# QZ1-boy/FCVSR

Measured on AMD Instinct MI355X. Metric: SR frames/sec (7-frame window, 4x 180x320->720x1280) + PSNR vs ref, higher is better.
Workload: dtype bf16

## Files before the change

### fcvsr_amd/csrc/convblk.hip

```cpp
#include "common.h"

namespace fcvsr {

constexpr int kCbT = 16;

template <int K>
__global__ __launch_bounds__(256) void convblk_conv_kernel(const float4* x, const float* __restrict__ w1,
                                                           const float* __restrict__ w2, const float* slope_p, float4* u,
                                                           float4* partial, int H, int W, int tiles_x, int tiles_y) {
  constexpr int P = K / 2;
  constexpr int XS = kCbT + 4 * P, TT = kCbT + 2 * P;
  __shared__ float4 xs[XS * XS];
  __shared__ float4 ts[TT * TT];
  __shared__ float4 red[256];
  const int tid = threadIdx.x;
  const int n = blockIdx.y;
  const int ty0 = (blockIdx.x / tiles_x) * kCbT, tx0 = (blockIdx.x % tiles_x) * kCbT;
  const float4* xn = x + (long long)n * H * W;
  const float slope = slope_p[0];
  for (int idx = tid; idx < XS * XS; idx += 256) {
    const int yy = idx / XS, xx = idx - yy * XS;
    const int gy = ty0 - 2 * P + yy, gx = tx0 - 2 * P + xx;
    float4 v = make_float4(0.f, 0.f, 0.f, 0.f);
    if (gy >= 0 && gy < H && gx >= 0 && gx < W) v = xn[(long long)gy * W + gx];
// ... 98 lines not shown
    gate_s[tid] = 1.f / (1.f + expf(-a));
  }
  __syncthreads();
  const long long pix = (long long)blockIdx.x * 256 + tid;
  if (pix >= HW) return;
  const int dir = bn / B, b = bn - dir * B;
  const float4 uu = u[(long long)bn * HW + pix];
  const float4 ss = sim[(long long)b * HW + pix];
  const float o0 = fmaf(uu.x, gate_s[0], uu.x) * ss.x;
  const float o1 = fmaf(uu.y, gate_s[1], uu.y) * ss.y;
  const float o2 = fmaf(uu.z, gate_s[2], uu.z) * ss.z;
  const float o3 = fmaf(uu.w, gate_s[3], uu.w) * ss.w;
  float* px = spec + ((long long)b * HW + pix) * ps;
  const int gi = (g0 + dir * g_stride) * 2;
  if (((ps | re_off | im_off) & 1) == 0 && (reinterpret_cast<uintptr_t>(spec) & 7) == 0) {
    *reinterpret_cast<float2*>(px + re_off + gi) = make_float2(o0, o1);
    *reinterpret_cast<float2*>(px + im_off + gi) = make_float2(o2, o3);
  } else {
    px[re_off + gi] = o0;
    px[re_off + gi + 1] = o1;
    px[im_off + gi] = o2;
    px[im_off + gi + 1] = o3;
  }
}

template <int K>
static void launch_convblk_conv(dim3 grid, hipStream_t st, const float4* x, const float* w1, const float* w2, const float* slope,
                                float4* u, float4* partial, int H, int W, int tx, int ty) {
  hipLaunchKernelGGL(convblk_conv_kernel<K>, grid, dim3(256), 0, st, x, w1, w2, slope, u, partial, H, W, tx, ty);
}

}

using namespace fcvsr;

extern "C" int fcvsr_convblk(const float* x, const float* w1, const float* w2, const float* prelu_slope, int ksize,
                             const float* ca_w1, const float* ca_w2, const float* sim, int B, int ndir, int H, int Wf,
                             float* u_scratch, float* partial_scratch, int64_t partial_elems, float* spec, int64_t pix_stride,
                             int re_off, int im_off, int g_stride, int g0, void* stream) {
  FCVSR_CHECK_ARG(x && w1 && w2 && prelu_slope && ca_w1 && ca_w2 && sim && u_scratch && partial_scratch && spec, "null pointer");
  FCVSR_CHECK_ARG(B > 0 && ndir > 0 && H > 0 && Wf > 0, "bad sizes");
  FCVSR_CHECK_ARG(ksize % 2 == 1 && ksize >= 1 && ksize <= 11, "kernel size: odd, 1..11");
  FCVSR_CHECK_ARG(((uintptr_t)x % 16) == 0 && ((uintptr_t)u_scratch % 16) == 0 && ((uintptr_t)sim % 16) == 0 &&
                      ((uintptr_t)partial_scratch % 16) == 0, "16-byte alignment");
  const int tx = cdiv(Wf, kCbT), ty = cdiv(H, kCbT);
  const int nblk = tx * ty, N = ndir * B;
  FCVSR_CHECK_ARG(partial_elems >= 4ll * N * nblk, "partial scratch too small");
  hipStream_t st = (hipStream_t)stream;
  dim3 grid(nblk, N);
  const float4* x4 = (const float4*)x;
  float4* u4 = (float4*)u_scratch;
  float4* p4 = (float4*)partial_scratch;
  switch (ksize) {
    case 1: launch_convblk_conv<1>(grid, st, x4, w1, w2, prelu_slope, u4, p4, H, Wf, tx, ty); break;
    case 3: launch_convblk_conv<3>(grid, st, x4, w1, w2, prelu_slope, u4, p4, H, Wf, tx, ty); break;
    case 5: launch_convblk_conv<5>(grid, st, x4, w1, w2, prelu_slope, u4, p4, H, Wf, tx, ty); break;
    case 7: launch_convblk_conv<7>(grid, st, x4, w1, w2, prelu_slope, u4, p4, H, Wf, tx, ty); break;
    case 9: launch_convblk_conv<9>(grid, st, x4, w1, w2, prelu_slope, u4, p4, H, Wf, tx, ty); break;
    default: launch_convblk_conv<11>(grid, st, x4, w1, w2, prelu_slope, u4, p4, H, Wf, tx, ty); break;
  }
  FCVSR_LAUNCH_CHECK();
  const long long HW = (long long)H * Wf;
  hipLaunchKernelGGL(convblk_tail_kernel2, dim3(cdiv(HW, 256), N), dim3(256), 0, st, (const float4*)u4, (const float4*)p4, nblk,
                     1.0f / (float)HW, ca_w1, ca_w2, (const float4*)sim, B, HW, spec, (long long)pix_stride, re_off, im_off,
                     g_stride, g0);
  FCVSR_LAUNCH_CHECK();
  return 0;
}
```

### fcvsr_amd/csrc/freq_head.hip

```cpp
#include "common.h"
#include "mfma_util.h"

namespace fcvsr {

constexpr int kFhPix = 128, kFhLD = 64 + 8;

struct FreqHeadArgs {
  const void* x;
  long long sx;
  float* out;
  int npix;
  const uint16_t* w0;
  const uint16_t* w1;
  const uint16_t* wl;
};

template <bool SRC_F32, int NHID>
__global__ __launch_bounds__(256, 4) void freq_head_kernel(FreqHeadArgs a) {
  __shared__ __align__(16) uint16_t A_s[kFhPix * kFhLD];
  __shared__ __align__(16) uint16_t B_s[64 * kFhLD];
  const int tid = threadIdx.x;
  const int lane = tid & 63, wave = tid >> 6;
  const int r = lane & 31, h = lane >> 5;
  const int flat0 = blockIdx.x * kFhPix;
  const int npix = a.npix;
  f32x16_t acc[2];
  auto zero_acc = [&]() {
#pragma unroll
    for (int nf = 0; nf < 2; ++nf)
#pragma unroll
      for (int i = 0; i < 16; ++i) acc[nf][i] = 0.f;
  };
  auto stage_w = [&](const uint16_t* w, int cin_pad, int c0, int rows) {
    uint4 v[2];
#pragma unroll
    for (int u = 0; u < 2; ++u) {
      const int row = (tid >> 3) + 32 * u;
      v[u] = make_uint4(0, 0, 0, 0);
      if (row < rows) v[u] = *reinterpret_cast<const uint4*>(w + (long long)row * cin_pad + c0 + (tid & 7) * 8);
    }
#pragma unroll
    for (int u = 0; u < 2; ++u) *reinterpret_cast<uint4*>(B_s + ((tid >> 3) + 32 * u) * kFhLD + (tid & 7) * 8) = v[u];
  };
  auto mma_chunk = [&](const uint16_t* prow, int ntile) {
    const uint16_t* wrow = B_s + r * kFhLD + h * 8;
#pragma unroll
    for (int kk = 0; kk < 4; ++kk) {
      const uint4 pf = *reinterpret_cast<const uint4*>(prow + kk * 16);
#pragma unroll
      for (int nf = 0; nf < 2; ++nf)
        if (nf < ntile) acc[nf] = mfma<true>(*reinterpret_cast<const uint4*>(wrow + nf * 32 * kFhLD + kk * 16), pf, acc[nf]);
    }
  };
  auto store_hidden = [&]() {
    uint16_t* trow = A_s + (wave * 32 + r) * kFhLD;
#pragma unroll
    for (int nf = 0; nf < 2; ++nf)
#pragma unroll
      for (int g = 0; g < 4; ++g) {
        const float4 v = make_float4(fmaxf(acc[nf][4 * g], 0.f), fmaxf(acc[nf][4 * g + 1], 0.f), fmaxf(acc[nf][4 * g + 2], 0.f),
                                     fmaxf(acc[nf][4 * g + 3], 0.f));
        *reinterpret_cast<uint2*>(trow + nf * 32 + 8 * g + 4 * h) = cvt4<true>(v);
      }
  };

  zero_acc();
  for (int c0 = 0; c0 < 128; c0 += 64) {
    __syncthreads();
    if (SRC_F32) {
      const int q = tid & 15, p0 = tid >> 4;
      const float* sb = reinterpret_cast<const float*>(a.x) + c0 + q * 4;
      float4 v[8];
#pragma unroll
      for (int i = 0; i < 8; ++i) {
        int pix = flat0 + p0 + i * 16;
        pix = pix < npix ? pix : npix - 1;
        v[i] = *reinterpret_cast<const float4*>(sb + (long long)pix * a.sx);
      }
#pragma unroll
      for (int i = 0; i < 8; ++i) *reinterpret_cast<uint2*>(A_s + (p0 + i * 16) * kFhLD + q * 4) = cvt4<true>(v[i]);
    } else {
      const int q = tid & 7, p0 = tid >> 3;
      const uint16_t* sb = reinterpret_cast<const uint16_t*>(a.x) + c0 + q * 8;
      uint4 v[4];
#pragma unroll
      for (int i = 0; i < 4; ++i) {
        int pix = flat0 + p0 + i * 32;
        pix = pix < npix ? pix : npix - 1;
        v[i] = *reinterpret_cast<const uint4*>(sb + (long long)pix * a.sx);
      }
#pragma unroll
      for (int i = 0; i < 4; ++i) *reinterpret_cast<uint4*>(A_s + (p0 + i * 32) * kFhLD + q * 8) = v[i];
    }
    stage_w(a.w0, 128, c0, 64);
    __syncthreads();
    mma_chunk(A_s + (wave * 32 + r) * kFhLD + h * 8, 2);
  }
  __syncthreads();
  store_hidden();

  if (NHID == 2) {
    zero_acc();
    __syncthreads();
    stage_w(a.w1, 64, 0, 64);
    __syncthreads();
    mma_chunk(A_s + (wave * 32 + r) * kFhLD + h * 8, 2);
    __builtin_amdgcn_wave_barrier();
    store_hidden();
  }

  zero_acc();
  __syncthreads();
  stage_w(a.wl, 64, 0, 32);
  __syncthreads();
  mma_chunk(A_s + (wave * 32 + r) * kFhLD + h * 8, 1);
  const int pix = flat0 + wave * 32 + r;
  if (h == 0 && pix < npix)
    *reinterpret_cast<float4*>(a.out + (long long)pix * 4) = make_float4(acc[0][0], acc[0][1], acc[0][2], acc[0][3]);
}

}

using namespace fcvsr;

extern "C" int fcvsr_freq_head(const void* x, int x_dtype, int64_t x_pix_stride, int64_t npix, const void* w0, const void* w_mid,
                               const void* w_last, float* out, void* stream) {
  FCVSR_CHECK_ARG(x && w0 && w_last && out, "null argument");
  FCVSR_CHECK_ARG(x_dtype == FCVSR_F32 || x_dtype == FCVSR_BF16, "x: f32 or bf16");
  FCVSR_CHECK_ARG(npix > 0 && npix < (1ll << 30) && x_pix_stride >= 128 && x_pix_stride % 8 == 0, "bad sizes / strides");
  FCVSR_CHECK_ARG(((uintptr_t)x % 16) == 0 && ((uintptr_t)w0 % 16) == 0 && ((uintptr_t)w_last % 16) == 0 &&
                      ((uintptr_t)out % 16) == 0 && (w_mid == nullptr || ((uintptr_t)w_mid % 16) == 0), "16-byte alignment");
  FreqHeadArgs a;
  a.x = x; a.sx = x_pix_stride; a.out = out; a.npix = (int)npix;
  a.w0 = (const uint16_t*)w0; a.w1 = (const uint16_t*)w_mid; a.wl = (const uint16_t*)w_last;
  dim3 grid(cdiv(npix, kFhPix));
  hipStream_t st = (hipStream_t)stream;
  if (x_dtype == FCVSR_F32) {
    if (w_mid) hipLaunchKernelGGL((freq_head_kernel<true, 2>), grid, dim3(256), 0, st, a);
    else hipLaunchKernelGGL((freq_head_kernel<true, 1>), grid, dim3(256), 0, st, a);
  } else {
    if (w_mid) hipLaunchKernelGGL((freq_head_kernel<false, 2>), grid, dim3(256), 0, st, a);
    else hipLaunchKernelGGL((freq_head_kernel<false, 1>), grid, dim3(256), 0, st, a);
  }
  FCVSR_LAUNCH_CHECK();
  return 0;
}
```

### fcvsr_amd/csrc/freq_mlp.hip

```cpp
#include "common.h"
#include "mfma_util.h"

namespace fcvsr {

constexpr int kFmC = 128;
constexpr int kFmPix = 128;
constexpr int kFmLD = 64 + 8;
constexpr int kFmTD = kFmC + 8;
constexpr int kFmTBytes = kFmPix * kFmTD * 2;
constexpr int kFmBBytes = kFmC * kFmLD * 2;
constexpr int kFmLds = kFmTBytes + kFmBBytes;

struct FreqMlpArgs {
  const float* xa[2];
  const float* xb[2];
  uint16_t* dst[2];
  long long sx, dsx;
  int npix, n_groups, tiles_per_group;
  const uint16_t* w0;
  const uint16_t* w2;
  const uint16_t* w4;
};

__global__ __launch_bounds__(256, 3) void freq_mlp3_kernel(FreqMlpArgs a) {
  extern __shared__ __align__(16) unsigned char lds[];
  uint16_t* T_s = reinterpret_cast<uint16_t*>(lds);
  uint16_t* A_s = T_s;
  uint16_t* B_s = reinterpret_cast<uint16_t*>(lds + kFmTBytes);
  const int tid = threadIdx.x;
  const int lane = tid & 63, wave = tid >> 6;
  const int r = lane & 31, h = lane >> 5;
  const int gi = blockIdx.x / a.tiles_per_group;
  const int flat0 = (blockIdx.x - gi * a.tiles_per_group) * kFmPix;
  const float* xa = a.xa[gi];
  const float* xb = a.xb[gi];
  const int npix = a.npix;

  f32x16_t acc[4];
  auto zero_acc = [&]() {
#pragma unroll
    for (int nf = 0; nf < 4; ++nf)
#pragma unroll
      for (int i = 0; i < 16; ++i) acc[nf][i] = 0.f;
  };
  auto mma_chunk = [&](const uint16_t* prow) {
    const uint16_t* wrow = B_s + r * kFmLD + h * 8;
#pragma unroll
    for (int kk = 0; kk < 4; ++kk) {
      const uint4 pf = *reinterpret_cast<const uint4*>(prow + kk * 16);
      uint4 wf[4];
#pragma unroll
      for (int nf = 0; nf < 4; ++nf) wf[nf] = *reinterpret_cast<const uint4*>(wrow + nf * 32 * kFmLD + kk * 16);
#pragma unroll
      for (int nf = 0; nf < 4; ++nf) acc[nf] = mfma<true>(wf[nf], pf, acc[nf]);
      if (kk & 1) __builtin_amdgcn_sched_barrier(0);
    }
// ... 138 lines not shown
                      dst_pix_stride >= kFmC && dst_pix_stride % 8 == 0, "bad sizes / strides");
  FCVSR_CHECK_ARG(npix * src_pix_stride * 4 < (1ll << 32) && npix * dst_pix_stride * 2 < (1ll << 32), "tensor too large for 32-bit offsets");
  FCVSR_CHECK_ARG(((uintptr_t)w0 % 16) == 0 && ((uintptr_t)w2 % 16) == 0 && ((uintptr_t)w4 % 16) == 0, "weights 16-byte aligned");
  FreqMlpArgs a;
  for (int d = 0; d < 2; ++d) {
    const int s = d < n_dirs ? d : 0;
    FCVSR_CHECK_ARG(xa[s] && xb[s] && dst[s] && ((uintptr_t)xa[s] % 16) == 0 && ((uintptr_t)xb[s] % 16) == 0 &&
                        ((uintptr_t)dst[s] % 16) == 0, "spectra / destination must be 16-byte aligned");
    a.xa[d] = xa[s]; a.xb[d] = xb[s]; a.dst[d] = (uint16_t*)dst[s];
  }
  a.sx = src_pix_stride; a.dsx = dst_pix_stride; a.npix = (int)npix; a.n_groups = n_dirs;
  a.tiles_per_group = cdiv(npix, kFmPix);
  a.w0 = (const uint16_t*)w0; a.w2 = (const uint16_t*)w2; a.w4 = (const uint16_t*)w4;
  static DevOnce attr;
  {
    hipError_t e = once_per_device(attr, [&] {
      return hipFuncSetAttribute((const void*)freq_mlp3_kernel, hipFuncAttributeMaxDynamicSharedMemorySize, kFmLds);
    });
    if (e != hipSuccess) {
      set_error("fcvsr_freq_mlp3: %s", hipGetErrorString(e));
      return (int)e;
    }
  }
  hipLaunchKernelGGL(freq_mlp3_kernel, dim3(a.tiles_per_group * n_dirs), dim3(256), kFmLds, (hipStream_t)stream, a);
  FCVSR_LAUNCH_CHECK();
  return 0;
}
```

### fcvsr_amd/engine.py

```python
from __future__ import annotations

import ctypes as C
import math
import weakref
from collections import OrderedDict
from typing import Dict, List, Optional, Tuple

import numpy as np
import torch

from . import hip
from .hip import ACT_LEAKY, ACT_NONE, ACT_PRELU, ACT_RELU, check, lib, ptr, stream_ptr, view


_MASKS: Dict[Tuple[int, int, int], torch.Tensor] = {}


def band_masks_half(Q: int, H: int, W: int) -> torch.Tensor:
    key = (Q, H, W)
    if key not in _MASKS:
        n = 1024
        step = math.sqrt((n / 2) ** 2 + (n / 2) ** 2) / Q
        d2 = (np.arange(-(n // 2), n - n // 2, 1) ** 2).astype(np.float64)
        r2 = np.power(np.sqrt(d2[:, None] + d2[None, :]), 2)
# ... 259 lines not shown
            cv = view(corr)
            check(L.fcvsr_corr_lookup(x1f.data_ptr(), x2f.data_ptr(), fs, B, H, Wf, 2 * n, 4, Wf, C.byref(cv), st),
                  "fcvsr_corr_lookup")
            for d in range(2):
                self._conv("MGAA.convcorr.0", [off[d * B:(d + 1) * B], corr], c0[d * B:(d + 1) * B], act=ACT_RELU, freq=True)
            self._conv("MGAA.convcorr.2", [c0], c1, act=ACT_RELU, freq=True)
            self._conv("MGAA.convcorr.4", [c1], off4, freq=True)
        else:
            if fused:
                check(L.fcvsr_freq_head(off.data_ptr(), hip.BF16, 2 * n, 2 * B * H * Wf,
                                        self._weights("MGAA.convcorr.0", torch.bfloat16, cols=(0, 2 * n))[0].data_ptr(),
                                        self._weights("MGAA.convcorr.2", torch.bfloat16)[0].data_ptr(),
                                        self._weights("MGAA.convcorr.4", torch.bfloat16)[0].data_ptr(), off4.data_ptr(), st),
                      "fcvsr_freq_head(convcorr)")
            else:
                c0 = self._new(dev, 2 * B, H, Wf, n, dtype=fdt)
                c1 = self._new(dev, 2 * B, H, Wf, n, dtype=fdt)
                self._conv("MGAA.convcorr.0", [off], c0, act=ACT_RELU, freq=True, cols=(0, 2 * n))
            xs = min(Wf, 8)
            corr = self._new(dev, B, H, xs, 84)
            cv = view(corr)
            check(L.fcvsr_corr_lookup(x1f.data_ptr(), x2f.data_ptr(), fs, B, H, Wf, 2 * n, 4, xs, C.byref(cv), st),
                  "fcvsr_corr_lookup")
            off_s = off[:, :, :xs].to(torch.float32, memory_format=torch.contiguous_format)
            c0_s = self._new(dev, 2 * B, H, xs, n, dtype=fdt)
            for d in range(2):
                self._conv("MGAA.convcorr.0", [off_s[d * B:(d + 1) * B], corr], c0_s[d * B:(d + 1) * B], act=ACT_RELU,
                           freq=True)
            if fused:
                c1_s = self._new(dev, 2 * B, H, xs, n, dtype=fdt)
                off4_s = self._new(dev, 2 * B, H, xs, 4)
                self._conv("MGAA.convcorr.2", [c0_s], c1_s, act=ACT_RELU, freq=True)
                self._conv("MGAA.convcorr.4", [c1_s], off4_s, freq=True)
                off4[:, :, :xs].copy_(off4_s)
            else:
                c0[:, :, :xs].copy_(c0_s)
                self._conv("MGAA.convcorr.2", [c0], c1, act=ACT_RELU, freq=True)
                self._conv("MGAA.convcorr.4", [c1], off4, freq=True)

        ospec = self._new(dev, B, H, Wf, 8 * A)
        u = self._new(dev, 2 * B, H, Wf, 4)
        ntile = ((H + 15) // 16) * ((Wf + 15) // 16)
        partial = self._new(dev, 2 * B * ntile * 4)
        for i in range(A):
            pre = f"MGAA.MConvB.{i}"
            w1 = self._weights(pre + ".conv1", "direct")[0]
            w2 = self._weights(pre + ".conv2", "direct")[0]
            check(L.fcvsr_convblk(off4.data_ptr(), w1.data_ptr(), w2.data_ptr(), par[pre + ".relu.weight"].data_ptr(),
                                  par[pre + ".conv1.weight"].shape[-1], par[pre + ".CA.conv_du.0.weight"].data_ptr(),
                                  par[pre + ".CA.conv_du.2.weight"].data_ptr(), sim.data_ptr(), B, 2, H, Wf, u.data_ptr(),
                                  partial.data_ptr(), partial.numel(), ospec.data_ptr(), 8 * A, 0, 4 * A, A, i, st),
                  "fcvsr_convblk")
        offsets = self._new(dev, B, H, W, 4 * A)
        ov = view(offsets)
        check(L.fcvsr_irfft2(ospec.data_ptr(), 8 * A, 4 * A, 0, B, H, W, 4 * A, None, None, C.byref(ov), st),
              "fcvsr_irfft2")

        kp = self._new(dev, B, H, W, n, dtype=self._adt())
        k0 = self._new(dev, B, H, W, n, dtype=self._adt())
        fused_iac = n % 32 == 0
        self._conv("MGAA.conv_KP", [x2], kp)
        self._conv("MGAA.F.0", [kp], k0)
        fold_f1 = fused_iac and n == 64 and self.precision != "f32" and self._model().fold_f1
        if not fold_f1:
            K = self._new(dev, B, H, W, A * 3 * n, dtype=self._adt() if fused_iac else torch.float32)
            self._conv("MGAA.F.1", [k0], K)

        fdt_act = x1.dtype
        al = self._new(dev, B, H, W, 2 * n, dtype=fdt_act)
        ping = [self._new(dev, B, H, W, n, dtype=fdt_act), self._new(dev, B, H, W, n, dtype=fdt_act)]
        if not fused_iac:
            if fdt_act != torch.float32:
                raise RuntimeError("16-bit activations need the fused IAC kernel (n_features % 32 == 0)")
            s = self._new(dev, B, H, W, n)
            vbuf = self._new(dev, B, H, W, n)
# ... 520 lines not shown
```

### fcvsr_amd/hip.py

```python
from __future__ import annotations

import ctypes as C
import os
from typing import Optional, Sequence

import numpy as np
import torch

_HERE = os.path.dirname(os.path.abspath(__file__))
LIB_PATH = os.path.join(_HERE, "lib", "libfcvsr_hip.so")

F32, BF16, F16, U8, U16 = 0, 1, 2, 3, 4
ACT_NONE, ACT_RELU, ACT_LEAKY, ACT_PRELU = 0, 1, 2, 3
_DT = {torch.float32: F32, torch.bfloat16: BF16, torch.float16: F16, torch.uint8: U8, torch.uint16: U16}


class View(C.Structure):
    _fields_ = [("ptr", C.c_void_p), ("sb", C.c_int64), ("sy", C.c_int64), ("sx", C.c_int64), ("sc", C.c_int64),
                ("c", C.c_int32), ("dtype", C.c_int32)]


class GcFinishLevel(C.Structure):
    _fields_ = [("partial", C.c_void_p), ("add", C.c_void_p), ("nparts", C.c_int32)]

# ... 62 lines not shown
    "fcvsr_last_conv_kernel": [],
    "fcvsr_conv2d_wgrad_scratch_elems": [C.c_int] * 7,
    "fcvsr_conv2d_wgrad": [C.c_void_p, C.c_void_p, C.c_int, C.c_int, C.c_int, C.c_int, C.c_int, C.c_int, C.c_int, C.c_void_p, C.c_void_p,
                           C.c_longlong, C.c_int, C.c_void_p],
    "fcvsr_conv2d_wgrad_mfma_eligible": [C.c_int] * 6,
    "fcvsr_conv2d_wgrad_mfma_scratch_elems": [C.c_int] * 7,
    "fcvsr_conv2d_wgrad_mfma": [C.c_void_p, C.c_void_p, C.c_int, C.c_int, C.c_int, C.c_int, C.c_int, C.c_int, C.c_int, C.c_void_p, C.c_void_p,
                                C.c_void_p, C.c_longlong, C.c_int, C.c_int, C.c_void_p],
    "fcvsr_abi_version": [],
    "fcvsr_device_count": [],
    "fcvsr_conv2d": [C.POINTER(ConvDesc), _VP],
    "fcvsr_conv2d_f32mfma": [C.POINTER(ConvDesc), _VP],
    "fcvsr_conv2d_f32mfma_eligible": [C.POINTER(ConvDesc)],
    "fcvsr_conv2d_mfma": [C.POINTER(ConvDesc), _I, _I, _VP],
    "fcvsr_conv2d_mfma_plan": [C.POINTER(ConvDesc), _I, _I, _I, _I, C.c_char_p, _I],
    "fcvsr_rfft2": [_PV, _I, _I, _I, _I, _VP, _I64, _I, _I, _VP],
    "fcvsr_irfft2": [_VP, _I64, _I, _I, _I, _I, _I, _I, _VP, _VP, _PV, _VP],
    "fcvsr_irfft2_bands": [_VP, _I64, _I, _I, _I, _I, _I, _I, _VP, _I, _VP, _PV, _VP],
    "fcvsr_corr_lookup": [_VP, _VP, _I64, _I, _I, _I, _I, _I, _I, _PV, _VP],
    "fcvsr_channel_sum": [_PV, _I, _I, _I, _VP, _VP, _I64, _VP],
    "fcvsr_ca_gate": [_VP, _F, _VP, _VP, _I, _I, _I, _VP, _VP],
    "fcvsr_convblk_tail": [_VP, _VP, _VP, _I, _I, _I, _I, _VP, _I64, _I, _I, _I, _I, _VP],
    "fcvsr_convblk": [_VP, _VP, _VP, _VP, _I, _VP, _VP, _VP, _I, _I, _I, _I, _VP, _VP, _I64, _VP, _I64, _I, _I, _I, _I, _VP],
    "fcvsr_warp": [_PV, _PV, _I, _I, _I, _PV, _VP],
    "fcvsr_sac_v": [_PV, _PV, _I, _I, _I, _PV, _VP],
    "fcvsr_sac_h": [_PV, _PV, _PV, _F, _I, _I, _I, _PV, _VP],
    "fcvsr_iac_step": [_PV, _PV, _PV, _PV, _F, _I, _I, _I, _PV, _VP],
    "fcvsr_feat_extract": [_PV, _I, _I, _I, _VP, _VP, _I, _VP, _VP, _VP, _I, _VP],
    "fcvsr_freq_head": [_VP, _I, _I64, _I64, _VP, _VP, _VP, _VP, _VP],
    "fcvsr_freq_mlp3": [_VP, _VP, _I, _I64, _I64, _VP, _VP, _VP, _VP, _I64, _VP],
    "fcvsr_iac_step2": [_PV, _PV, _PV, _PV, _F, _I, _I, _I, _PV, _VP],
    "fcvsr_iac_step2_fused": [_PV, _PV, _PV, _VP, _VP, _PV, _F, _I, _I, _I, _PV, _VP],
    "fcvsr_divenh": [_I, _I, _VP, _VP, _VP, _VP, _VP, _VP, _F, _VP, _VP, _VP, _VP, _I64, _I, _I, _I, _I, _VP],
    "fcvsr_divenh_apply_next": [_I, _VP, _VP, _VP, _VP, _VP, _VP, _F, _VP, _VP, _VP, _VP, _VP, _VP, _VP, _I64, _I, _I, _I, _I, _VP],
    "fcvsr_divenh_stage": [C.POINTER(DivEnhStageArgs), _VP],
    "fcvsr_scale_add": [_VP, _VP, _VP, _I, _VP, _I, _I, _I, _I, _I, _VP],
    "fcvsr_gc_context": [_VP, _VP, _VP, _VP, _I, _I, _I, _I, _VP, _VP, _I64, _VP],
    "fcvsr_gc_finish": [_VP, _I, _VP, _VP, _I, _I, _VP, _VP],
    "fcvsr_gc_apply": [_VP, _VP, _VP, _VP, _I, _F, _I, _I, _I, _I, _VP],
    "fcvsr_xscale": [_VP, _VP, _F, _VP, _VP, _VP, _I, _I, _I, _I, _I, _VP],
    "fcvsr_gc_finish_levels": [C.POINTER(GcFinishLevel), _I, _VP, _VP, _I, _I, _VP],
    "fcvsr_gc_partial_levels": [C.POINTER(GcPartialLevel), _I, _I, _VP, _I, _VP],
    "fcvsr_gc_apply_levels": [C.POINTER(GcApplyLevel), _I, _I, _I, _F, _I, _VP],
    "fcvsr_xscale_levels": [C.POINTER(XscaleLevel), _I, _I, _I, _VP],
    "fcvsr_rcb_level0": [_VP, _VP, _VP, _VP, _VP, _VP, _VP, _F, _F, _I, _I, _I, _I, _I, _VP],
    "fcvsr_rcb_tail": [C.POINTER(RcbTailArgs), _F, _I, _I, _VP],
    "fcvsr_pixel_shuffle": [_VP, _VP, _I, _I, _I, _I, _VP],
    "fcvsr_pixel_shuffle16": [_VP, _PV, _I, _I, _I, _I, _VP],
    "fcvsr_bilinear_up4": [_PV, _I, _I, _I, _PV, _VP],
    "fcvsr_tail_fused": [_PV, _VP, _VP, _VP, _VP, _VP, _I, _I, _I, _PV, _VP],
    "fcvsr_tail_fused_base": [_PV, _VP, _VP, _VP, _VP, _VP, _PV, _I, _I, _I, _PV, _VP],
    "fcvsr_conv_last": [_PV, _VP, _VP, _I, _I, _I, _I, _PV, _VP],
# ... 347 lines not shown
```

### include/fcvsr_hip.h

```cpp
#ifndef FCVSR_HIP_H
#define FCVSR_HIP_H

#include <stddef.h>
#include <stdint.h>

#ifdef __cplusplus
extern "C" {
#endif

#define FCVSR_ABI_VERSION 2

enum { FCVSR_E_ARG = -1, FCVSR_E_UNSUPPORTED = -2, FCVSR_E_NOGPU = -3 };
enum { FCVSR_F32 = 0, FCVSR_BF16 = 1, FCVSR_F16 = 2 };
enum { FCVSR_U8 = 3 };
enum { FCVSR_U16 = 4 };
enum { FCVSR_ACT_NONE = 0, FCVSR_ACT_RELU = 1, FCVSR_ACT_LEAKY = 2, FCVSR_ACT_PRELU = 3 };

typedef struct fcvsr_view {
  void*   ptr;
  int64_t sb, sy, sx, sc;
  int32_t c;
  int32_t dtype;
} fcvsr_view;

// ... 85 lines not shown
int fcvsr_rfft2(const fcvsr_view* src, int B, int H, int W, int n,
                float* spec, int64_t pix_stride, int im_off, int re_off, void* stream);
int fcvsr_irfft2(const float* spec, int64_t pix_stride, int im_off, int re_off, int B, int H, int W, int n,
                 const float* mask, float* work, const fcvsr_view* dst, void* stream);
int fcvsr_irfft2_bands(const float* spec, int64_t pix_stride, int im_off, int re_off, int B, int H, int W, int n,
                       const float* masks, int n_bands, float* work, const fcvsr_view* dst, void* stream);

int fcvsr_feat_extract(const fcvsr_view* x, int B, int H, int W, const void* w, const float* bias, int n_blk,
                       void* const* dst, const int64_t* dst_pix_stride, const int32_t* dst_ch_off, int dst_dtype,
                       void* stream);

int fcvsr_corr_lookup(const float* x1f, const float* x2f, int64_t pix_stride, int B, int H, int Wf, int C, int radius,
                      int x_count, const fcvsr_view* dst, void* stream);
int fcvsr_channel_sum(const fcvsr_view* src, int B, int H, int W, float* out, float* scratch, int64_t scratch_elems,
                      void* stream);
int fcvsr_ca_gate(const float* sum, float inv_hw, const float* w1, const float* w2, int B, int c, int cr,
                  float* gate, void* stream);
int fcvsr_convblk_tail(const float* u, const float* gate, const float* sim, int B, int ndir, int H, int Wf,
                       float* spec, int64_t pix_stride, int re_off, int im_off, int g_stride, int g0, void* stream);
int fcvsr_convblk(const float* x, const float* w1, const float* w2, const float* prelu_slope, int ksize, const float* ca_w1,
                  const float* ca_w2, const float* sim, int B, int ndir, int H, int Wf, float* u_scratch,
                  float* partial_scratch, int64_t partial_elems, float* spec, int64_t pix_stride, int re_off, int im_off,
                  int g_stride, int g0, void* stream);
int fcvsr_warp(const fcvsr_view* src, const fcvsr_view* off, int B, int H, int W, const fcvsr_view* dst, void* stream);
int fcvsr_sac_v(const fcvsr_view* s, const fcvsr_view* k1, int B, int H, int W, const fcvsr_view* dst, void* stream);
int fcvsr_sac_h(const fcvsr_view* v, const fcvsr_view* k1, const fcvsr_view* feat_in, float slope,
                int B, int H, int W, const fcvsr_view* dst, void* stream);

int fcvsr_iac_step(const fcvsr_view* prev, const fcvsr_view* off, const fcvsr_view* k1, const fcvsr_view* feat_in,
                   float slope, int B, int H, int W, const fcvsr_view* dst, void* stream);
int fcvsr_iac_step2(const fcvsr_view* prev, const fcvsr_view* off, const fcvsr_view* k1, const fcvsr_view* feat_in,
                    float slope, int B, int H, int W, const fcvsr_view* dst, void* stream);
int fcvsr_iac_step2_fused(const fcvsr_view* prev, const fcvsr_view* off, const fcvsr_view* k0, const void* wk,
                          const float* kbias, const fcvsr_view* feat_in, float slope, int B, int H, int W,
                          const fcvsr_view* dst, void* stream);

int fcvsr_freq_mlp3(const float* const* xa, const float* const* xb, int n_dirs, int64_t src_pix_stride, int64_t npix,
                    const void* w0, const void* w2, const void* w4, void* const* dst, int64_t dst_pix_stride, void* stream);

int fcvsr_freq_head(const void* x, int x_dtype, int64_t x_pix_stride, int64_t npix, const void* w0, const void* w_mid,
                    const void* w_last, float* out, void* stream);

int fcvsr_divenh(int mode, int first, const float* f, float* s_f, float* s_o, const float* a, const float* b,
                 const float* mean_f_sum, float inv_hw, const float* g1, const float* g2,
                 float* sums, float* scratch, int64_t scratch_elems, int B, int H, int W, int C, void* stream);
int fcvsr_divenh_apply_next(int first, const float* f, float* s_f, float* s_o, const float* a, const float* b,
                            const float* mean_f_sum, float inv_hw, const float* g1, const float* g2,
                            const float* f_next, const float* a_next, const float* b_next, float* sums,
                            float* scratch, int64_t scratch_elems, int B, int H, int W, int C, void* stream);
typedef struct {
  const float* ck_s_f;
  const float* ck_s_o;
  const float* f[4];
  const float* a[4];
  const float* b[4];
  const float* g1[4];
  const float* g2[4];
  const float* mean_f_sum;
  const float* f_next;
  const float* a_next;
  const float* b_next;
  float*       out_s_f;
  float*       out_s_o;
  float*       sums;
// ... 138 lines not shown
```

Baseline: 913.5.

## Fuse MConvB heads into one kernel and convcorr strip into one MLP kernel

All A MConvB heads are now computed in one conv kernel that loads the input tile once with the largest halo, plus one tail kernel that applies every head's channel-attention gate and writes all heads' spectrum records with float4 stores. This replaces 2*A launches. The convcorr path, which used a dtype-conversion copy, several conv launches and a strip copy, becomes a single bf16 MFMA freq_head variant. That variant reads the offset spectra and the correlation volume directly and writes into the full-width off4. The freq_mlp3 grid is also remapped to interleave the two directions in groups of eight tiles. The cost is a larger u/partial scratch, a larger LDS halo per block, and more templated code paths.

New measurement: 930.1, median of 6. 1.02x the previous value.

```diff
diff --git a/fcvsr_amd/csrc/convblk.hip b/fcvsr_amd/csrc/convblk.hip
--- a/fcvsr_amd/csrc/convblk.hip
+++ b/fcvsr_amd/csrc/convblk.hip
@@ -144,6 +144,207 @@
     px[im_off + gi] = o2;
     px[im_off + gi + 1] = o3;
   }
+}
+
+constexpr int kCbMaxHeads = 6;
+typedef const __attribute__((address_space(4))) float cb_cfloat_t;
+__device__ __forceinline__ cb_cfloat_t* cb_const(const float* p) { return reinterpret_cast<cb_cfloat_t*>(reinterpret_cast<uintptr_t>(p)); }
+
+struct ConvBlkHeadsArgs {
+  const float* w1[kCbMaxHeads];
+  const float* w2[kCbMaxHeads];
+  const float* slope[kCbMaxHeads];
+  const float* ca_w1[kCbMaxHeads];
+  const float* ca_w2[kCbMaxHeads];
+};
+
+template <int A, int I>
+__device__ __forceinline__ void convblk_one_head(const float4* xs, float4* ts, float4* red, cb_cfloat_t* w1, cb_cfloat_t* w2, float slope, float4* __restrict__ un,
+                                                 float4* __restrict__ partial_out, int H, int W, int ty0, int tx0, int tid) {
+  constexpr int K = 2 * I + 1, P = I;
+  constexpr int XS = kCbT + 4 * (A - 1), TT = kCbT + 2 * P;
+  constexpr int D = 2 * (A - 1) - 2 * P;
+  for (int idx = tid; idx < TT * TT; idx += 256) {
+    const int yy = idx / TT, xx = idx - yy * TT;
+    const int gy = ty0 - P + yy, gx = tx0 - P + xx;
+    float a0 = 0.f, a1 = 0.f, a2 = 0.f, a3 = 0.f;
+    if (gy >= 0 && gy < H && gx >= 0 && gx < W) {
+#pragma unroll
+      for (int ky = 0; ky < K; ++ky) {
+#pragma unroll
+        for (int kx = 0; kx < K; ++kx) {
+          const float4 v = xs[(yy + ky + D) * XS + xx + kx + D];
+          cb_cfloat_t* wt = w1 + (ky * K + kx) * 64;
+          const float vi[4] = {v.x, v.y, v.z, v.w};
+#pragma unroll
+          for (int ci = 0; ci < 4; ++ci) {
+            a0 = fmaf(vi[ci], wt[ci * 16 + 0], a0); a1 = fmaf(vi[ci], wt[ci * 16 + 1], a1);
+            a2 = fmaf(vi[ci], wt[ci * 16 + 2], a2); a3 = fmaf(vi[ci], wt[ci * 16 + 3], a3);
+          }
+        }
+      }
+      a0 = a0 >= 0.f ? a0 : a0 * slope; a1 = a1 >= 0.f ? a1 : a1 * slope;
+      a2 = a2 >= 0.f ? a2 : a2 * slope; a3 = a3 >= 0.f ? a3 : a3 * slope;
+    }
+    ts[idx] = make_float4(a0, a1, a2, a3);
+  }
+  __syncthreads();
+  const int ly = tid >> 4, lx = tid & 15;
+  const int gy = ty0 + ly, gx = tx0 + lx;
+  float4 o = make_float4(0.f, 0.f, 0.f, 0.f);
+  if (gy < H && gx < W) {
+    float a0 = 0.f, a1 = 0.f, a2 = 0.f, a3 = 0.f;
+#pragma unroll
+    for (int ky = 0; ky < K; ++ky) {
+#pragma unroll
+      for (int kx = 0; kx < K; ++kx) {
+        const float4 v = ts[(ly + ky) * TT + lx + kx];
+        cb_cfloat_t* wt = w2 + (ky * K + kx) * 64;
+        const float vi[4] = {v.x, v.y, v.z, v.w};
+#pragma unroll
+        for (int ci = 0; ci < 4; ++ci) {
+          a0 = fmaf(vi[ci], wt[ci * 16 + 0], a0); a1 = fmaf(vi[ci], wt[ci * 16 + 1], a1);
+          a2 = fmaf(vi[ci], wt[ci * 16 + 2], a2); a3 = fmaf(vi[ci], wt[ci * 16 + 3], a3);
+        }
+      }
+    }
+    o = make_float4(a0, a1, a2, a3);
+    un[(long long)gy * W + gx] = o;
+  }
+  red[tid] = o;
+  __syncthreads();
+  for (int st = 128; st > 0; st >>= 1) {
+    if (tid < st) {
+      const float4 p = red[tid], q = red[tid + st];
+      red[tid] = make_float4(p.x + q.x, p.y + q.y, p.z + q.z, p.w + q.w);
+    }
+    __syncthreads();
+  }
+  if (tid == 0) *partial_out = red[0];
+}
+
+template <int A, int I>
+__device__ __forceinline__ void convblk_heads_from(const float4* xs, float4* ts, float4* red, const ConvBlkHeadsArgs& a, float4* u,
+                                                   float4* partial, int N, int n, int H, int W, int ty0, int tx0, int tid) {
+  convblk_one_head<A, I>(xs, ts, red, cb_const(a.w1[I]), cb_const(a.w2[I]), cb_const(a.slope[I])[0], u + ((long long)I * N + n) * H * W,
+                         partial + ((long long)I * N + n) * gridDim.x + blockIdx.x, H, W, ty0, tx0, tid);
+  if constexpr (I + 1 < A) convblk_heads_from<A, I + 1>(xs, ts, red, a, u, partial, N, n, H, W, ty0, tx0, tid);
+}
+
+template <int A>
+__global__ __launch_bounds__(256) void convblk_heads_conv_kernel(const float4* x, ConvBlkHeadsArgs a, float4* u, float4* partial,
+                                                                 int N, int H, int W, int tiles_x) {
+  constexpr int PM = 2 * (A - 1);
+  constexpr int XS = kCbT + 2 * PM, TT = kCbT + PM;
+  __shared__ float4 xs[XS * XS];
+  __shared__ float4 ts[TT * TT];
+  __shared__ float4 red[256];
+  const int tid = threadIdx.x;
+  const int n = blockIdx.y;
+  const int ty0 = (blockIdx.x / tiles_x) * kCbT, tx0 = (blockIdx.x % tiles_x) * kCbT;
+  const float4* xn = x + (long long)n * H * W;
+  for (int idx = tid; idx < XS * XS; idx += 256) {
+    const int yy = idx / XS, xx = idx - yy * XS;
+    const int gy = ty0 - PM + yy, gx = tx0 - PM + xx;
+    float4 v = make_float4(0.f, 0.f, 0.f, 0.f);
+    if (gy >= 0 && gy < H && gx >= 0 && gx < W) v = xn[(long long)gy * W + gx];
+    xs[idx] = v;
+  }
+  __syncthreads();
+  convblk_heads_from<A, 0>(xs, ts, red, a, u, partial, N, n, H, W, ty0, tx0, tid);
+}
+
+template <int A>
+__global__ __launch_bounds__(256) void convblk_heads_tail_kernel(const float4* __restrict__ u, const float4* __restrict__ partial,
+                                                                 int nblk, float inv_hw, ConvBlkHeadsArgs a,
+                                                                 const float4* __restrict__ sim, int B, long long HW,
+                                                                 float* __restrict__ spec, long long ps, int re_off, int im_off) {
+  constexpr int NP = 2 * A;
+  __shared__ float4 red[NP][256];
+  __shared__ float gate_s[NP][4];
+  const int tid = threadIdx.x;
+  const int b = blockIdx.y;
+  const long long pix = (long long)blockIdx.x * 256 + tid;
+  const bool live = pix < HW;
+  float4 uu[NP], ss = make_float4(0.f, 0.f, 0.f, 0.f);
+#pragma unroll
+  for (int p = 0; p < NP; ++p) {
+    const long long bn = (long long)(p % A) * 2 * B + (p / A) * B + b;
+    uu[p] = make_float4(0.f, 0.f, 0.f, 0.f);
+    if (live) uu[p] = u[bn * HW + pix];
+  }
+  if (live) ss = sim[(long long)b * HW + pix];
+#pragma unroll
+  for (int p = 0; p < NP; ++p) {
+    const long long bn = (long long)(p % A) * 2 * B + (p / A) * B + b;
+    float4 s = make_float4(0.f, 0.f, 0.f, 0.f);
+    for (int k = tid; k < nblk; k += 256) {
+      const float4 q = partial[bn * nblk + k];
+      s = make_float4(s.x + q.x, s.y + q.y, s.z + q.z, s.w + q.w);
+    }
+    red[p][tid] = s;
+  }
+  __syncthreads();
+  for (int st = 128; st > 0; st >>= 1) {
+    if (tid < st) {
+#pragma unroll
+      for (int p = 0; p < NP; ++p) {
+        const float4 q0 = red[p][tid], q1 = red[p][tid + st];
+        red[p][tid] = make_float4(q0.x + q1.x, q0.y + q1.y, q0.z + q1.z, q0.w + q1.w);
+      }
+    }
+    __syncthreads();
+  }
+#pragma unroll
+  for (int p = 0; p < NP; ++p) {
+    if ((tid >> 2) == p) {
+      const float* ca_w1 = a.ca_w1[p % A];
+      const float* ca_w2 = a.ca_w2[p % A];
+      const int row = tid & 3;
+      const float4 t = red[p][0];
+      const float mean[4] = {t.x * inv_hw, t.y * inv_hw, t.z * inv_hw, t.w * inv_hw};
+      float hid[4];
+#pragma unroll
+      for (int h = 0; h < 4; ++h) {
+        float acc = 0.f;
+#pragma unroll
+        for (int c = 0; c < 4; ++c) acc = fmaf(ca_w1[h * 4 + c], mean[c], acc);
+        hid[h] = fmaxf(acc, 0.f);
+      }
+      float acc = 0.f;
+#pragma unroll
+      for (int h = 0; h < 4; ++h) acc = fmaf(ca_w2[row * 4 + h], hid[h], acc);
+      gate_s[p][row] = 1.f / (1.f + expf(-acc));
+    }
+  }
+  __syncthreads();
+  if (!live) return;
+  float o[NP][4];
+#pragma unroll
+  for (int p = 0; p < NP; ++p) {
+    o[p][0] = fmaf(uu[p].x, gate_s[p][0], uu[p].x) * ss.x;
+    o[p][1] = fmaf(uu[p].y, gate_s[p][1], uu[p].y) * ss.y;
+    o[p][2] = fmaf(uu[p].z, gate_s[p][2], uu[p].z) * ss.z;
+    o[p][3] = fmaf(uu[p].w, gate_s[p][3], uu[p].w) * ss.w;
+  }
+  float* px = spec + ((long long)b * HW + pix) * ps;
+#pragma unroll
+  for (int q = 0; q < A; ++q)
+    *reinterpret_cast<float4*>(px + re_off + 4 * q) = make_float4(o[2 * q][0], o[2 * q][1], o[2 * q + 1][0], o[2 * q + 1][1]);
+#pragma unroll
+  for (int q = 0; q < A; ++q)
+    *reinterpret_cast<float4*>(px + im_off + 4 * q) = make_float4(o[2 * q][2], o[2 * q][3], o[2 * q + 1][2], o[2 * q + 1][3]);
+}
+
+template <int A>
+static void launch_convblk_heads(hipStream_t st, const float4* x, const ConvBlkHeadsArgs& a, float4* u, float4* partial,
+                                 const float4* sim, int B, int H, int W, float* spec, long long ps, int re_off, int im_off) {
+  const int tx = cdiv(W, kCbT), ty = cdiv(H, kCbT);
+  const int nblk = tx * ty, N = 2 * B;
+  const long long HW = (long long)H * W;
+  hipLaunchKernelGGL(convblk_heads_conv_kernel<A>, dim3(nblk, N), dim3(256), 0, st, x, a, u, partial, N, H, W, tx);
+  hipLaunchKernelGGL(convblk_heads_tail_kernel<A>, dim3(cdiv(HW, 256), B), dim3(256), 0, st, (const float4*)u,
+                     (const float4*)partial, nblk, 1.0f / (float)HW, a, sim, B, HW, spec, ps, re_off, im_off);
 }
 
 template <int K>
@@ -189,3 +390,40 @@
   FCVSR_LAUNCH_CHECK();
   return 0;
 }
+
+extern "C" int fcvsr_convblk_heads(const float* x, int n_heads, const float* const* w1, const float* const* w2,
+                                   const float* const* prelu_slope, const float* const* ca_w1, const float* const* ca_w2,
+                                   const float* sim, int B, int H, int Wf, float* u, float* partial, int64_t partial_elems,
+                                   float* spec, int64_t pix_stride, int re_off, int im_off, void* stream) {
+  FCVSR_CHECK_ARG(x && w1 && w2 && prelu_slope && ca_w1 && ca_w2 && sim && u && partial && spec, "null pointer");
+  FCVSR_CHECK_ARG(n_heads >= 1 && n_heads <= kCbMaxHeads, "heads: 1..6");
+  FCVSR_CHECK_ARG(B > 0 && H > 0 && Wf > 0, "bad sizes");
+  FCVSR_CHECK_ARG(((uintptr_t)x % 16) == 0 && ((uintptr_t)u % 16) == 0 && ((uintptr_t)sim % 16) == 0 &&
+                      ((uintptr_t)partial % 16) == 0 && ((uintptr_t)spec % 16) == 0, "16-byte alignment");
+  FCVSR_CHECK_ARG(pix_stride % 4 == 0 && re_off % 4 == 0 && im_off % 4 == 0 && re_off >= 0 && im_off >= 0 &&
+                      re_off + 4 * n_heads <= pix_stride && im_off + 4 * n_heads <= pix_stride &&
+                      (re_off + 4 * n_heads <= im_off || im_off + 4 * n_heads <= re_off), "record: two disjoint 16-byte aligned blocks");
+  const long long nblk = (long long)cdiv(Wf, kCbT) * cdiv(H, kCbT);
+  FCVSR_CHECK_ARG(partial_elems >= 4ll * n_heads * 2 * B * nblk, "partial scratch too small");
+  ConvBlkHeadsArgs a = {};
+  for (int i = 0; i < n_heads; ++i) {
+    FCVSR_CHECK_ARG(w1[i] && w2[i] && prelu_slope[i] && ca_w1[i] && ca_w2[i], "null head pointer");
+    a.w1[i] = w1[i]; a.w2[i] = w2[i]; a.slope[i] = prelu_slope[i]; a.ca_w1[i] = ca_w1[i]; a.ca_w2[i] = ca_w2[i];
+  }
+  hipStream_t st = (hipStream_t)stream;
+  const float4* x4 = (const float4*)x;
+  const float4* s4 = (const float4*)sim;
+  float4* u4 = (float4*)u;
+  float4* p4 = (float4*)partial;
+  const long long ps = (long long)pix_stride;
+  switch (n_heads) {
+    case 1: launch_convblk_heads<1>(st, x4, a, u4, p4, s4, B, H, Wf, spec, ps, re_off, im_off); break;
+    case 2: launch_convblk_heads<2>(st, x4, a, u4, p4, s4, B, H, Wf, spec, ps, re_off, im_off); break;
+    case 3: launch_convblk_heads<3>(st, x4, a, u4, p4, s4, B, H, Wf, spec, ps, re_off, im_off); break;
+    case 4: launch_convblk_heads<4>(st, x4, a, u4, p4, s4, B, H, Wf, spec, ps, re_off, im_off); break;
+    case 5: launch_convblk_heads<5>(st, x4, a, u4, p4, s4, B, H, Wf, spec, ps, re_off, im_off); break;
+    default: launch_convblk_heads<6>(st, x4, a, u4, p4, s4, B, H, Wf, spec, ps, re_off, im_off); break;
+  }
+  FCVSR_LAUNCH_CHECK();
+  return 0;
+}
diff --git a/fcvsr_amd/csrc/freq_head.hip b/fcvsr_amd/csrc/freq_head.hip
--- a/fcvsr_amd/csrc/freq_head.hip
+++ b/fcvsr_amd/csrc/freq_head.hip
@@ -13,10 +13,13 @@
   const uint16_t* w0;
   const uint16_t* w1;
   const uint16_t* wl;
+  const float* corr;
+  int xs, Wf, corr_npix;
 };
 
-template <bool SRC_F32, int NHID>
+template <bool SRC_F32, int NHID, bool STRIP = false>
 __global__ __launch_bounds__(256, 4) void freq_head_kernel(FreqHeadArgs a) {
+  static_assert(!STRIP || (!SRC_F32 && NHID == 2), "the strip variant is convcorr on the bf16 offset spectra");
   __shared__ __align__(16) uint16_t A_s[kFhPix * kFhLD];
   __shared__ __align__(16) uint16_t B_s[64 * kFhLD];
   const int tid = threadIdx.x;
@@ -42,10 +45,11 @@
 #pragma unroll
     for (int u = 0; u < 2; ++u) *reinterpret_cast<uint4*>(B_s + ((tid >> 3) + 32 * u) * kFhLD + (tid & 7) * 8) = v[u];
   };
-  auto mma_chunk = [&](const uint16_t* prow, int ntile) {
+  auto mma_chunk = [&](const uint16_t* prow, int ntile, int nk = 4) {
     const uint16_t* wrow = B_s + r * kFhLD + h * 8;
 #pragma unroll
     for (int kk = 0; kk < 4; ++kk) {
+      if (STRIP && kk >= nk) break;
       const uint4 pf = *reinterpret_cast<const uint4*>(prow + kk * 16);
 #pragma unroll
       for (int nf = 0; nf < 2; ++nf)
@@ -64,10 +68,32 @@
       }
   };
 
+  auto grid_pix = [&](int pix) -> long long {
+    if (!STRIP) return pix;
+    const int row = pix / a.xs;
+    return (long long)row * a.Wf + (pix - row * a.xs);
+  };
   zero_acc();
-  for (int c0 = 0; c0 < 128; c0 += 64) {
+  constexpr int CIN0 = STRIP ? 256 : 128;
+  for (int c0 = 0; c0 < CIN0; c0 += 64) {
     __syncthreads();
-    if (SRC_F32) {
+    if (STRIP && c0 >= 128) {
+      const int q = tid & 15, p0 = tid >> 4;
+      const int c = c0 - 128 + q * 4;
+      const float* sb = a.corr + (c < 84 ? c : 0);
+      float4 v[8];
+#pragma unroll
+      for (int i = 0; i < 8; ++i) {
+        int pix = flat0 + p0 + i * 16;
+        pix = pix < npix ? pix : npix - 1;
+        v[i] = *reinterpret_cast<const float4*>(sb + (long long)(pix % a.corr_npix) * 84);
+      }
+#pragma unroll
+      for (int i = 0; i < 8; ++i) {
+        if (c >= 84) v[i] = make_float4(0.f, 0.f, 0.f, 0.f);
+        *reinterpret_cast<uint2*>(A_s + (p0 + i * 16) * kFhLD + q * 4) = cvt4<true>(v[i]);
+      }
+    } else if (SRC_F32) {
       const int q = tid & 15, p0 = tid >> 4;
       const float* sb = reinterpret_cast<const float*>(a.x) + c0 + q * 4;
       float4 v[8];
@@ -87,14 +113,14 @@
       for (int i = 0; i < 4; ++i) {
         int pix = flat0 + p0 + i * 32;
         pix = pix < npix ? pix : npix - 1;
-        v[i] = *reinterpret_cast<const uint4*>(sb + (long long)pix * a.sx);
+        v[i] = *reinterpret_cast<const uint4*>(sb + grid_pix(pix) * a.sx);
       }
 #pragma unroll
       for (int i = 0; i < 4; ++i) *reinterpret_cast<uint4*>(A_s + (p0 + i * 32) * kFhLD + q * 8) = v[i];
     }
-    stage_w(a.w0, 128, c0, 64);
+    stage_w(a.w0, CIN0, c0, 64);
     __syncthreads();
-    mma_chunk(A_s + (wave * 32 + r) * kFhLD + h * 8, 2);
+    mma_chunk(A_s + (wave * 32 + r) * kFhLD + h * 8, 2, c0 == 192 ? 2 : 4);
   }
   __syncthreads();
   store_hidden();
@@ -116,7 +142,7 @@
   mma_chunk(A_s + (wave * 32 + r) * kFhLD + h * 8, 1);
   const int pix = flat0 + wave * 32 + r;
   if (h == 0 && pix < npix)
-    *reinterpret_cast<float4*>(a.out + (long long)pix * 4) = make_float4(acc[0][0], acc[0][1], acc[0][2], acc[0][3]);
+    *reinterpret_cast<float4*>(a.out + grid_pix(pix) * 4) = make_float4(acc[0][0], acc[0][1], acc[0][2], acc[0][3]);
 }
 
 }
@@ -130,7 +156,7 @@
   FCVSR_CHECK_ARG(npix > 0 && npix < (1ll << 30) && x_pix_stride >= 128 && x_pix_stride % 8 == 0, "bad sizes / strides");
   FCVSR_CHECK_ARG(((uintptr_t)x % 16) == 0 && ((uintptr_t)w0 % 16) == 0 && ((uintptr_t)w_last % 16) == 0 &&
                       ((uintptr_t)out % 16) == 0 && (w_mid == nullptr || ((uintptr_t)w_mid % 16) == 0), "16-byte alignment");
-  FreqHeadArgs a;
+  FreqHeadArgs a = {};
   a.x = x; a.sx = x_pix_stride; a.out = out; a.npix = (int)npix;
   a.w0 = (const uint16_t*)w0; a.w1 = (const uint16_t*)w_mid; a.wl = (const uint16_t*)w_last;
   dim3 grid(cdiv(npix, kFhPix));
@@ -145,3 +171,19 @@
   FCVSR_LAUNCH_CHECK();
   return 0;
 }
+
+extern "C" int fcvsr_convcorr_strip(const void* off, const float* corr, int B, int H, int Wf, int xs, const void* w0,
+                                    const void* w_mid, const void* w_last, float* off4, void* stream) {
+  FCVSR_CHECK_ARG(off && corr && w0 && w_mid && w_last && off4, "null argument");
+  FCVSR_CHECK_ARG(B > 0 && H > 0 && Wf > 0 && xs > 0 && xs <= Wf && 2ll * B * H * Wf < (1ll << 30), "bad sizes");
+  FCVSR_CHECK_ARG(((uintptr_t)off % 16) == 0 && ((uintptr_t)corr % 16) == 0 && ((uintptr_t)w0 % 16) == 0 &&
+                      ((uintptr_t)w_mid % 16) == 0 && ((uintptr_t)w_last % 16) == 0 && ((uintptr_t)off4 % 16) == 0,
+                  "16-byte alignment");
+  FreqHeadArgs a = {};
+  a.x = off; a.sx = 128; a.out = off4; a.npix = 2 * B * H * xs;
+  a.w0 = (const uint16_t*)w0; a.w1 = (const uint16_t*)w_mid; a.wl = (const uint16_t*)w_last;
+  a.corr = corr; a.xs = xs; a.Wf = Wf; a.corr_npix = B * H * xs;
+  hipLaunchKernelGGL((freq_head_kernel<false, 2, true>), dim3(cdiv(a.npix, kFhPix)), dim3(256), 0, (hipStream_t)stream, a);
+  FCVSR_LAUNCH_CHECK();
+  return 0;
+}
diff --git a/fcvsr_amd/csrc/freq_mlp.hip b/fcvsr_amd/csrc/freq_mlp.hip
--- a/fcvsr_amd/csrc/freq_mlp.hip
+++ b/fcvsr_amd/csrc/freq_mlp.hip
@@ -30,8 +30,16 @@
   const int tid = threadIdx.x;
   const int lane = tid & 63, wave = tid >> 6;
   const int r = lane & 31, h = lane >> 5;
-  const int gi = blockIdx.x / a.tiles_per_group;
-  const int flat0 = (blockIdx.x - gi * a.tiles_per_group) * kFmPix;
+  int gi, tile;
+  if (a.n_groups == 2) {
+    tile = (blockIdx.x >> 4) * 8 + (blockIdx.x & 7);
+    gi = (blockIdx.x >> 3) & 1;
+    if (tile >= a.tiles_per_group) return;
+  } else {
+    gi = 0;
+    tile = blockIdx.x;
+  }
+  const int flat0 = tile * kFmPix;
   const float* xa = a.xa[gi];
   const float* xb = a.xb[gi];
   const int npix = a.npix;
@@ -216,7 +224,7 @@
       return (int)e;
     }
   }
-  hipLaunchKernelGGL(freq_mlp3_kernel, dim3(a.tiles_per_group * n_dirs), dim3(256), kFmLds, (hipStream_t)stream, a);
+  hipLaunchKernelGGL(freq_mlp3_kernel, dim3(n_dirs == 2 ? cdiv(a.tiles_per_group, 8) * 16 : a.tiles_per_group), dim3(256), kFmLds, (hipStream_t)stream, a);
   FCVSR_LAUNCH_CHECK();
   return 0;
 }
diff --git a/fcvsr_amd/engine.py b/fcvsr_amd/engine.py
--- a/fcvsr_amd/engine.py
+++ b/fcvsr_amd/engine.py
@@ -305,35 +305,46 @@
             cv = view(corr)
             check(L.fcvsr_corr_lookup(x1f.data_ptr(), x2f.data_ptr(), fs, B, H, Wf, 2 * n, 4, xs, C.byref(cv), st),
                   "fcvsr_corr_lookup")
-            off_s = off[:, :, :xs].to(torch.float32, memory_format=torch.contiguous_format)
-            c0_s = self._new(dev, 2 * B, H, xs, n, dtype=fdt)
-            for d in range(2):
-                self._conv("MGAA.convcorr.0", [off_s[d * B:(d + 1) * B], corr], c0_s[d * B:(d + 1) * B], act=ACT_RELU,
-                           freq=True)
             if fused:
-                c1_s = self._new(dev, 2 * B, H, xs, n, dtype=fdt)
-                off4_s = self._new(dev, 2 * B, H, xs, 4)
-                self._conv("MGAA.convcorr.2", [c0_s], c1_s, act=ACT_RELU, freq=True)
-                self._conv("MGAA.convcorr.4", [c1_s], off4_s, freq=True)
-                off4[:, :, :xs].copy_(off4_s)
+                check(L.fcvsr_convcorr_strip(off.data_ptr(), corr.data_ptr(), B, H, Wf, xs,
+                                             self._weights("MGAA.convcorr.0", torch.bfloat16)[0].data_ptr(),
+                                             self._weights("MGAA.convcorr.2", torch.bfloat16)[0].data_ptr(),
+                                             self._weights("MGAA.convcorr.4", torch.bfloat16)[0].data_ptr(), off4.data_ptr(), st),
+                      "fcvsr_convcorr_strip")
             else:
+                off_s = off[:, :, :xs].to(torch.float32, memory_format=torch.contiguous_format)
+                c0_s = self._new(dev, 2 * B, H, xs, n, dtype=fdt)
+                for d in range(2):
+                    self._conv("MGAA.convcorr.0", [off_s[d * B:(d + 1) * B], corr], c0_s[d * B:(d + 1) * B], act=ACT_RELU,
+                               freq=True)
                 c0[:, :, :xs].copy_(c0_s)
                 self._conv("MGAA.convcorr.2", [c0], c1, act=ACT_RELU, freq=True)
                 self._conv("MGAA.convcorr.4", [c1], off4, freq=True)
 
         ospec = self._new(dev, B, H, Wf, 8 * A)
-        u = self._new(dev, 2 * B, H, Wf, 4)
         ntile = ((H + 15) // 16) * ((Wf + 15) // 16)
-        partial = self._new(dev, 2 * B * ntile * 4)
-        for i in range(A):
-            pre = f"MGAA.MConvB.{i}"
-            w1 = self._weights(pre + ".conv1", "direct")[0]
-            w2 = self._weights(pre + ".conv2", "direct")[0]
-            check(L.fcvsr_convblk(off4.data_ptr(), w1.data_ptr(), w2.data_ptr(), par[pre + ".relu.weight"].data_ptr(),
-                                  par[pre + ".conv1.weight"].shape[-1], par[pre + ".CA.conv_du.0.weight"].data_ptr(),
-                                  par[pre + ".CA.conv_du.2.weight"].data_ptr(), sim.data_ptr(), B, 2, H, Wf, u.data_ptr(),
-                                  partial.data_ptr(), partial.numel(), ospec.data_ptr(), 8 * A, 0, 4 * A, A, i, st),
-                  "fcvsr_convblk")
+        heads = [f"MGAA.MConvB.{i}" for i in range(A)]
+        w1s = [self._weights(pre + ".conv1", "direct")[0] for pre in heads]
+        w2s = [self._weights(pre + ".conv2", "direct")[0] for pre in heads]
+        if A <= 6 and all(t.data_ptr() % 16 == 0 for t in (off4, sim, ospec)):
+            u = self._new(dev, A, 2 * B, H, Wf, 4)
+            partial = self._new(dev, A * 2 * B * ntile * 4)
+            PA = C.c_void_p * A
+            check(L.fcvsr_convblk_heads(off4.data_ptr(), A, PA(*[w.data_ptr() for w in w1s]), PA(*[w.data_ptr() for w in w2s]),
+                                        PA(*[par[pre + ".relu.weight"].data_ptr() for pre in heads]),
+                                        PA(*[par[pre + ".CA.conv_du.0.weight"].data_ptr() for pre in heads]),
+                                        PA(*[par[pre + ".CA.conv_du.2.weight"].data_ptr() for pre in heads]), sim.data_ptr(), B, H,
+                                        Wf, u.data_ptr(), partial.data_ptr(), partial.numel(), ospec.data_ptr(), 8 * A, 0, 4 * A,
+                                        st), "fcvsr_convblk_heads")
+        else:
+            u = self._new(dev, 2 * B, H, Wf, 4)
+            partial = self._new(dev, 2 * B * ntile * 4)
+            for i, pre in enumerate(heads):
+                check(L.fcvsr_convblk(off4.data_ptr(), w1s[i].data_ptr(), w2s[i].data_ptr(), par[pre + ".relu.weight"].data_ptr(),
+                                      par[pre + ".conv1.weight"].shape[-1], par[pre + ".CA.conv_du.0.weight"].data_ptr(),
+                                      par[pre + ".CA.conv_du.2.weight"].data_ptr(), sim.data_ptr(), B, 2, H, Wf, u.data_ptr(),
+                                      partial.data_ptr(), partial.numel(), ospec.data_ptr(), 8 * A, 0, 4 * A, A, i, st),
+                      "fcvsr_convblk")
         offsets = self._new(dev, B, H, W, 4 * A)
         ov = view(offsets)
         check(L.fcvsr_irfft2(ospec.data_ptr(), 8 * A, 4 * A, 0, B, H, W, 4 * A, None, None, C.byref(ov), st),
diff --git a/fcvsr_amd/hip.py b/fcvsr_amd/hip.py
--- a/fcvsr_amd/hip.py
+++ b/fcvsr_amd/hip.py
@@ -108,12 +108,14 @@
     "fcvsr_ca_gate": [_VP, _F, _VP, _VP, _I, _I, _I, _VP, _VP],
     "fcvsr_convblk_tail": [_VP, _VP, _VP, _I, _I, _I, _I, _VP, _I64, _I, _I, _I, _I, _VP],
     "fcvsr_convblk": [_VP, _VP, _VP, _VP, _I, _VP, _VP, _VP, _I, _I, _I, _I, _VP, _VP, _I64, _VP, _I64, _I, _I, _I, _I, _VP],
+    "fcvsr_convblk_heads": [_VP, _I, _VP, _VP, _VP, _VP, _VP, _VP, _I, _I, _I, _VP, _VP, _I64, _VP, _I64, _I, _I, _VP],
     "fcvsr_warp": [_PV, _PV, _I, _I, _I, _PV, _VP],
     "fcvsr_sac_v": [_PV, _PV, _I, _I, _I, _PV, _VP],
     "fcvsr_sac_h": [_PV, _PV, _PV, _F, _I, _I, _I, _PV, _VP],
     "fcvsr_iac_step": [_PV, _PV, _PV, _PV, _F, _I, _I, _I, _PV, _VP],
     "fcvsr_feat_extract": [_PV, _I, _I, _I, _VP, _VP, _I, _VP, _VP, _VP, _I, _VP],
     "fcvsr_freq_head": [_VP, _I, _I64, _I64, _VP, _VP, _VP, _VP, _VP],
+    "fcvsr_convcorr_strip": [_VP, _VP, _I, _I, _I, _I, _VP, _VP, _VP, _VP, _VP],
     "fcvsr_freq_mlp3": [_VP, _VP, _I, _I64, _I64, _VP, _VP, _VP, _VP, _I64, _VP],
     "fcvsr_iac_step2": [_PV, _PV, _PV, _PV, _F, _I, _I, _I, _PV, _VP],
     "fcvsr_iac_step2_fused": [_PV, _PV, _PV, _VP, _VP, _PV, _F, _I, _I, _I, _PV, _VP],
diff --git a/include/fcvsr_hip.h b/include/fcvsr_hip.h
--- a/include/fcvsr_hip.h
+++ b/include/fcvsr_hip.h
@@ -131,6 +131,10 @@
                   const float* ca_w2, const float* sim, int B, int ndir, int H, int Wf, float* u_scratch,
                   float* partial_scratch, int64_t partial_elems, float* spec, int64_t pix_stride, int re_off, int im_off,
                   int g_stride, int g0, void* stream);
+int fcvsr_convblk_heads(const float* x, int n_heads, const float* const* w1, const float* const* w2,
+                        const float* const* prelu_slope, const float* const* ca_w1, const float* const* ca_w2, const float* sim,
+                        int B, int H, int Wf, float* u, float* partial, int64_t partial_elems, float* spec, int64_t pix_stride,
+                        int re_off, int im_off, void* stream);
 int fcvsr_warp(const fcvsr_view* src, const fcvsr_view* off, int B, int H, int W, const fcvsr_view* dst, void* stream);
 int fcvsr_sac_v(const fcvsr_view* s, const fcvsr_view* k1, int B, int H, int W, const fcvsr_view* dst, void* stream);
 int fcvsr_sac_h(const fcvsr_view* v, const fcvsr_view* k1, const fcvsr_view* feat_in, float slope,
@@ -149,6 +153,8 @@
 
 int fcvsr_freq_head(const void* x, int x_dtype, int64_t x_pix_stride, int64_t npix, const void* w0, const void* w_mid,
                     const void* w_last, float* out, void* stream);
+int fcvsr_convcorr_strip(const void* off, const float* corr, int B, int H, int Wf, int xs, const void* w0, const void* w_mid,
+                         const void* w_last, float* off4, void* stream);
 
 int fcvsr_divenh(int mode, int first, const float* f, float* s_f, float* s_o, const float* a, const float* b,
                  const float* mean_f_sum, float inv_hw, const float* g1, const float* g2,
```
